# andfoy/py-distributed-dot-product

Hardware: AMD Instinct MI355X
Metric: ms/fwd+bwd DistributedDotProductAttn T=25000 d=768 h=8; scaling 1/2/4/8 GPU (lower is better)
Workload: dtype bf16; 1 GPU; model=DistributedDotProductAttn(d=768,h=8), global_batch=1, seq_len=25000, parallelism=sp1, impl=flash, mask=zeros, step=fwd+bwd+grad-allreduce+AdamW, launch=eager

## Files before the change

### csrc/bindings.cpp

```cpp
#include "bindings_common.h"

#include <algorithm>
#include <cmath>
#include <string>
#include <vector>

extern "C" const char xdot_build_id[];

using namespace xdot::bind;

namespace {

std::string build_id() { return std::string(xdot_build_id + 14); }

at::Tensor softmax_fwd(const at::Tensor& x, const c10::optional<at::Tensor>& mask, double scale,
                       int64_t mdiv, int64_t mmul, int64_t mmod) {
  Range rr_("xdot.softmax_fwd");
  TORCH_CHECK(x.is_cuda() && x.is_contiguous(), "xdot.softmax_fwd: x must be a contiguous GPU tensor");
  const int64_t T = x.size(-1);
  const int64_t rows = T == 0 ? 0 : x.numel() / T;
  auto y = at::empty_like(x);
  xdot::smx::Args a{};
  a.x = x.data_ptr(); a.out = y.data_ptr(); a.rows = rows; a.T = T; a.scale = (float)scale;
  a.mdiv = mdiv; a.mmul = mmul; a.mmod = mmod; a.mask = nullptr;
// ... 342 lines not shown
    hipKernelNodeAttrValue v{};
    v.priority = (int)prio;
    graph_ok(hipGraphKernelNodeSetAttribute(nd, hipKernelNodeAttributePriority, &v), "graph_set_kernel_priority");
    return;
  }
  TORCH_CHECK(false, "xdot.graph_set_kernel_priority: no kernel node ", index);
}

}

TORCH_LIBRARY(xdot, m) {
  m.def("gemm(Tensor A, Tensor B, Tensor(a!) C, int M, int N, int K, int nseg, int nb1, int nb2, "
        "int lda, int ldb, int ldc, int sA1, int sA2, int sB1, int sB2, int sC1, int sC2, "
        "int sAseg, int sBseg, bool a_mc, bool b_mc, float alpha, float beta=0.0, int path=0) -> ()");
  m.def("gemm_plan(int M, int N, int K, int nseg, int nb1, int nb2, int lda, int ldb, int ldc, int sA1, int sA2, "
        "int sB1, int sB2, int sC1, int sC2, int sAseg, int sBseg, bool a_mc, bool b_mc, float beta, ScalarType dt_in, "
        "ScalarType dt_out, bool a16, bool b16, bool c16, int path) -> int[]");
  m.def("softmax_fwd(Tensor x, Tensor? mask, float scale, int mdiv, int mmul, int mmod) -> Tensor");
  m.def("softmax_bwd(Tensor y, Tensor dy, float scale) -> Tensor");
  m.def("mask_pack(Tensor mask) -> (Tensor, Tensor, Tensor)");
  m.def("mask_gen(int B, int R, int T, bool causal, int window, int row_offset, Tensor? lengths, Tensor segs, Tensor? doc_starts=None, Tensor? row_runs=None) -> (Tensor, Tensor, Tensor)");
  m.def("flash_fwd(Tensor rows, Tensor kc, Tensor vc, Tensor? bits, Tensor? flags, int H, float scale, int nsplit=0, bool prescaled=False, int fp32_mode=0, Tensor(a!)? sbuf=None, int Hg=0) -> (Tensor, Tensor)");
  m.def("flash_bwd_cols(Tensor dout, Tensor rows, Tensor kc, Tensor vc, Tensor out, Tensor lse, Tensor? bits, "
        "Tensor? flags, int H, float scale, Tensor? delta=None, bool fp32_out=True, bool prescaled=False, "
        "Tensor? lse2=None, int fp32_mode=0, Tensor(a!)? sbuf=None, Tensor(b!)? dsbuf=None, int passes=3, "
        "Tensor(c!)? dkv_out=None, int Hg=0) -> (Tensor, Tensor)");
  m.def("flash_bwd_prep(Tensor dout, Tensor out, Tensor lse, int H) -> (Tensor, Tensor)");
  m.def("flash_bwd_delta(Tensor dout, Tensor out, int H) -> Tensor");
  m.def("sum_partials(Tensor part, ScalarType out_dtype) -> Tensor");
  m.def("flash_splits(int B, int R, int T, int H, bool rows_kernel) -> int");
  m.def("flash_fwd_plan(int B, int R, int T, int H, int D, ScalarType dtype, int fp32_mode, bool sbuf, int nsplit) -> int[]");
  m.def("flash_cols_plan(int B, int R, int T, int H, int D, ScalarType dtype, int fp32_mode, bool sbuf, bool dsbuf, "
        "int passes, bool prescaled, bool fp32_out, int Hg=0) -> int[]");
  m.def("flash_fwd_partial(Tensor rows, Tensor kc, Tensor vc, Tensor? bits, Tensor? flags, int H, float scale, "
        "Tensor(a!) opart, Tensor(b!) lpart, int sp0, int nsplit, bool prescaled=False, int fp32_mode=0, int Hg=0) -> ()");
  m.def("flash_fwd_combine(Tensor opart, Tensor lpart, int H, Tensor like) -> (Tensor, Tensor)");
  m.def("flash_bwd_rows_partial(Tensor dout, Tensor rows, Tensor kc, Tensor vc, Tensor lse, Tensor delta, Tensor? bits, "
        "Tensor? flags, int H, float scale, Tensor(a!) dpart, int sp0, int nsplit, bool prescaled=False, int fp32_mode=0, int Hg=0) -> ()");
  m.def("flash_bwd_rows_sum(Tensor dpart, int H, Tensor like) -> Tensor");
  m.def("flash_fwd_merge(Tensor(a!) opart, Tensor lpart, Tensor(b!) lrun, int H) -> ()");
  m.def("sum_partials_into(Tensor part, Tensor(a!) out) -> ()");
  m.def("cast_multi(Tensor[] src, Tensor(a!)[] dst) -> ()");
  m.def("adamw_step(Tensor(a!)[] params, Tensor[] grads, Tensor(b!)[] exp_avg, Tensor(c!)[] exp_avg_sq, float lr, "
        "float beta1, float beta2, float eps, float weight_decay, int step, Tensor[] step_ts, Tensor? lr_t, "
        "Tensor(d!)[] grad_out) -> ()");
  m.def("flash_bwd_rows(Tensor dout, Tensor rows, Tensor kc, Tensor vc, Tensor lse, Tensor delta, Tensor? bits, "
        "Tensor? flags, int H, float scale, int nsplit=0, bool prescaled=False, int fp32_mode=0, Tensor? sbuf=None, "
        "Tensor? dsbuf=None, int Hg=0) -> Tensor");
  m.def("flash_prescale(Tensor x, float scale) -> Tensor");
  m.def("rope_table(int R, int D, int offset, Tensor inv_freq) -> (Tensor, Tensor)");
  m.def("rope_apply(Tensor x, Tensor cos, Tensor sin, int H, bool inverse, float alpha, Tensor(a!) out) -> ()");
  m.def("headnorm_plan(int B, int R, int H, int D, ScalarType dtype) -> int[]");
  m.def("headnorm_fwd(Tensor x, Tensor weight, Tensor? cos, Tensor? sin, int H, float eps, float alpha, Tensor(a!) out, "
        "bool save) -> (Tensor, Tensor)");
  m.def("headnorm_bwd(Tensor g, Tensor x, Tensor rstd, Tensor weight, Tensor? cos, Tensor? sin, int H, float alpha, "
        "Tensor(a!) dx, bool need_dw) -> Tensor");
  m.def("sink_fold(Tensor(a!) out, Tensor(b!) lse, Tensor sinks, int H) -> ()");
  m.def("sink_grad(Tensor delta, Tensor lse, Tensor sinks) -> Tensor");
  m.def("gate_apply(Tensor o, Tensor g, int H, Tensor(a!) out, int mode=-1) -> ()");
  m.def("gate_backward(Tensor dy, Tensor o, Tensor g, int H, Tensor(a!) dout, int mode=-1) -> Tensor");
  m.def("mse_fwd(Tensor y, Tensor t) -> (Tensor, Tensor)");
  m.def("proj(Tensor x, Tensor w, Tensor? bias, bool nn, Tensor(a!)? out=None, int force=0, float alpha=1.0) -> Tensor");
  m.def("wgrad(Tensor dy, Tensor x, ScalarType out_dtype, int splits=0) -> Tensor");
  m.def("wgrad2(Tensor dy0, Tensor x0, Tensor dy1, Tensor x1, ScalarType out_dtype) -> Tensor[]");
  m.def("ipc_info() -> int[]");
  m.def("ipc_alloc(int nbytes, bool uncached) -> int");
// ... 43 lines not shown
```

### csrc/bindings_flash.cpp

```cpp
#include "bindings_common.h"
#include "flash_plan.h"

#include <vector>

namespace {

using namespace xdot::bind;
using namespace xdot::fa;
using OptT = c10::optional<at::Tensor>;

struct FlashGeom { int64_t B, R, C, T, D, ld, Cg, G; };

FlashGeom flash_check(const at::Tensor& rows, const at::Tensor& kc, const at::Tensor& vc, int64_t H, const OptT& bits,
                      const OptT& flags, bool colmajor = false, int64_t Hg = 0) {
  TORCH_CHECK(rows.is_cuda() && kc.is_cuda() && vc.is_cuda(), "xdot.flash: GPU tensors required");
  TORCH_CHECK(rows.is_contiguous(), "xdot.flash: rows must be contiguous");
  TORCH_CHECK(rows.scalar_type() == kc.scalar_type() && rows.scalar_type() == vc.scalar_type(), "xdot.flash: dtype mismatch");
  TORCH_CHECK(rows.scalar_type() == at::kBFloat16 || rows.scalar_type() == at::kHalf || rows.scalar_type() == at::kFloat,
              "xdot.flash: bf16/fp16/fp32 only");
  TORCH_CHECK(rows.dim() == 3 && kc.dim() == 3 && vc.sizes() == kc.sizes(), "xdot.flash: rows (B,R,C), cols (B,T,C)");
  FlashGeom g{rows.size(0), rows.size(1), rows.size(2), kc.size(1), 0, kc.stride(1), 0, 1};
  TORCH_CHECK(H > 0 && g.C % H == 0, "xdot.flash: C not divisible by heads");
  const int64_t hg = Hg > 0 ? Hg : H;
  TORCH_CHECK(hg <= H && H % hg == 0, "xdot.flash: the heads H = ", H, " must be a multiple of the gathered heads Hg = ", hg);
// ... 324 lines not shown
  Range rr_("xdot.flash_bwd_delta");
  return std::get<0>(bwd_prep(dout, out, nullptr, H, "flash_bwd_delta"));
}

std::tuple<at::Tensor, at::Tensor> flash_bwd_prep(const at::Tensor& dout, const at::Tensor& out, const at::Tensor& lse,
                                                  int64_t H) {
  Range rr_("xdot.flash_bwd_prep");
  return bwd_prep(dout, out, &lse, H, "flash_bwd_prep");
}

at::Tensor flash_bwd_rows(const at::Tensor& dout, const at::Tensor& rows, const at::Tensor& kc, const at::Tensor& vc,
                          const at::Tensor& lse, const at::Tensor& delta, const OptT& bits, const OptT& flags, int64_t H,
                          double scale, int64_t nsplit, bool prescaled, int64_t fp32_mode, const OptT& sbuf,
                          const OptT& dsbuf, int64_t Hg) {
  Range rr_("xdot.flash_bwd_rows");
  const FlashGeom g = flash_check(rows, kc, vc, H, bits, flags, false, Hg);
  float* sb = sbuf_ptr(sbuf, g, H, rows, fp32_mode, "xdot.flash_bwd_rows");
  float* dsb = sbuf_ptr(dsbuf, g, H, rows, fp32_mode, "xdot.flash_bwd_rows (dS buffer)");
  TORCH_CHECK(!dsb || sb || g.D <= 128, "xdot.flash_bwd_rows: a dS buffer without the score buffer needs D <= 128");
  check_bhr(delta, g.B, H, g.R, rows.device(), "xdot.flash_bwd_rows: delta");
  auto a = bwd_args(g, dout, rows, kc, vc, lse, bits, flags, H, scale, prescaled, fp32_mode);
  auto drows = at::empty_like(rows);
  const int ns = plan_rows(g, H, rows.scalar_type(), fp32_mode, sb || dsb, sb != nullptr, nsplit);
  at::Tensor dpart;
  if (ns > 1) dpart = at::empty({ns, g.B, g.R, g.C}, rows.options().dtype(at::kFloat));
  a.delta = delta.data_ptr<float>(); a.drows = drows.data_ptr();
  a.nsplit = ns; a.dpart = ns > 1 ? dpart.data_ptr<float>() : nullptr;
  a.sbuf = sb; a.dsbuf = dsb;
  c10::DeviceGuard guard(rows.device());
  launched(xdot_flash_bwd_rows_launch(&a, dt_code(rows.scalar_type()), (int)g.D, cur_stream(rows)), "flash_bwd_rows");
  return drows;
}

int64_t flash_splits(int64_t B, int64_t R, int64_t T, int64_t H, bool rows_kernel) {
  if (rows_kernel) return rows_split(B, R, T, H);
  return pick_split(((R + 127) / 128) * B * H, T, 512, 0);
}

void flash_fwd_partial(const at::Tensor& rows, const at::Tensor& kc, const at::Tensor& vc, const OptT& bits,
                       const OptT& flags, int64_t H, double scale, at::Tensor& opart, at::Tensor& lpart, int64_t sp0,
                       int64_t nsplit, bool prescaled, int64_t fp32_mode, int64_t Hg) {
  Range rr_("xdot.flash_fwd_partial");
  const FlashGeom g = flash_check(rows, kc, vc, H, bits, flags, false, Hg);
  TORCH_CHECK(sp0 >= 0 && nsplit >= 1, "xdot.flash_fwd_partial: slots");
  const int ns = pick_split(1, g.T, 1, nsplit);
  check_part(opart, sp0 + ns, g.B * g.R * g.C, "opart");
  check_part(lpart, sp0 + ns, g.B * H * g.R, "lpart");
  auto a = fwd_args(g, rows, kc, vc, bits, flags, H, scale, prescaled, fp32_mode);
  a.nsplit = ns; a.sp0 = (int)sp0; a.force_partial = 1;
  a.opart = opart.data_ptr<float>(); a.lpart = lpart.data_ptr<float>();
  c10::DeviceGuard guard(rows.device());
  launched(xdot_flash_fwd_launch(&a, dt_code(rows.scalar_type()), (int)g.D, cur_stream(rows)), "flash_fwd_partial");
}

void combine(xdot::fa::FwdArgs& a, const at::Tensor& opart, const at::Tensor& lpart, int64_t B, int64_t H, int64_t R,
             int64_t C, int dt, const char* op) {
  const int64_t S = opart.size(0);
  check_part(opart, S, B * R * C, "opart");
  check_part(lpart, S, B * H * R, "lpart");
  a.B = (int)B; a.H = (int)H; a.R = (int)R; a.nsplit = (int)S;
  a.opart = opart.data_ptr<float>(); a.lpart = lpart.data_ptr<float>();
  c10::DeviceGuard guard(opart.device());
  launched(xdot_flash_fwd_combine_launch(&a, dt, (int)(C / H), cur_stream(opart)), op);
}

std::tuple<at::Tensor, at::Tensor> flash_fwd_combine(const at::Tensor& opart, const at::Tensor& lpart, int64_t H,
// ... 29 lines not shown
  const FlashGeom g = flash_check(rows, kc, vc, H, bits, flags, false, Hg);
  check_bhr(delta, g.B, H, g.R, rows.device(), "xdot.flash_bwd_rows_partial: delta");
  TORCH_CHECK(sp0 >= 0 && nsplit >= 1, "xdot.flash_bwd_rows_partial: slots");
  const int ns = pick_split(1, g.T, 1, nsplit);
  check_part(dpart, sp0 + ns, g.B * g.R * g.C, "dpart");
  auto a = bwd_args(g, dout, rows, kc, vc, lse, bits, flags, H, scale, prescaled, fp32_mode);
  a.delta = delta.data_ptr<float>();
  a.nsplit = ns; a.sp0 = (int)sp0; a.force_partial = 1; a.dpart = dpart.data_ptr<float>();
  c10::DeviceGuard guard(rows.device());
  launched(xdot_flash_bwd_rows_launch(&a, dt_code(rows.scalar_type()), (int)g.D, cur_stream(rows)),
           "flash_bwd_rows_partial");
}

at::Tensor flash_bwd_rows_sum(const at::Tensor& dpart, int64_t H, const at::Tensor& like) {
  Range rr_("xdot.flash_bwd_rows_sum");
  const int64_t B = like.size(0), R = like.size(1), C = like.size(2), S = dpart.size(0);
  check_part(dpart, S, B * R * C, "dpart");
  auto out = at::empty_like(like);
  xdot::fa::BwdArgs a{};
  a.drows = out.data_ptr(); a.dpart = dpart.data_ptr<float>();
  a.B = (int)B; a.H = (int)H; a.R = (int)R; a.nsplit = (int)S;
  c10::DeviceGuard guard(like.device());
  launched(xdot_flash_bwd_rows_sum_launch(&a, dt_code(like.scalar_type()), (int)(C / H), cur_stream(like)),
           "flash_bwd_rows_sum");
  return out;
}

}

TORCH_LIBRARY_IMPL(xdot, CompositeExplicitAutograd, m) {
  m.impl("flash_splits", &flash_splits);
  m.impl("flash_fwd_plan", &flash_fwd_plan);
  m.impl("flash_cols_plan", &flash_cols_plan);
}

TORCH_LIBRARY_IMPL(xdot, CUDA, m) {
  m.impl("flash_fwd", &flash_fwd);
  m.impl("flash_bwd_cols", &flash_bwd_cols);
  m.impl("flash_bwd_rows", &flash_bwd_rows);
  m.impl("flash_bwd_delta", &flash_bwd_delta);
  m.impl("flash_bwd_prep", &flash_bwd_prep);
  m.impl("sum_partials", &sum_partials);
  m.impl("sum_partials_into", &sum_partials_into);
  m.impl("flash_prescale", &flash_prescale);
  m.impl("flash_fwd_partial", &flash_fwd_partial);
  m.impl("flash_fwd_combine", &flash_fwd_combine);
  m.impl("flash_fwd_merge", &flash_fwd_merge);
  m.impl("flash_bwd_rows_partial", &flash_bwd_rows_partial);
  m.impl("flash_bwd_rows_sum", &flash_bwd_rows_sum);
}
```

### csrc/flash_bwd.hip

```cpp
#include "flash_launch.h"

#include <algorithm>
#include <cstdlib>
#include <cstring>

#include <type_traits>

namespace xdot {
namespace fa {

template <int DT, int D>
__global__ __launch_bounds__(256) void flash_bwd_prep_kernel(BwdArgs a, const void* out_, float* delta) {
  using T16 = typename dt_traits<DT>::T;
  const int64_t idx = (int64_t)blockIdx.x * blockDim.x + threadIdx.x;
  const int64_t total = (int64_t)a.B * a.R * a.H;
  if (idx >= total) return;
  const int h = (int)(idx % a.H);
  const int64_t br = idx / a.H;
  const int row = (int)(br % a.R), b = (int)(br / a.R);
  const int64_t li = ((int64_t)b * a.H + h) * a.R + row;
  if (a.lse2) a.lse2[li] = a.lse[li] * LOG2E;
  if (!delta) return;
  const int64_t off = br * (a.H * D) + h * D;
  const T16* o = reinterpret_cast<const T16*>(out_) + off;
  const T16* d = reinterpret_cast<const T16*>(a.dout) + off;
  float acc = 0.f;
#pragma unroll
  for (int c = 0; c < D / 8; ++c) {
    union { u32x4 u; T16 e[8]; } x, y;
    x.u = *reinterpret_cast<const u32x4*>(o + 8 * c);
    y.u = *reinterpret_cast<const u32x4*>(d + 8 * c);
#pragma unroll
    for (int e = 0; e < 8; ++e) acc += (float)x.e[e] * (float)y.e[e];
  }
  delta[li] = acc;
// ... 537 lines not shown
template <int DT, int D>
static void launch_bwd_delta(const BwdArgs& a, const void* out, float* delta, hipStream_t st) {
  const int64_t n0 = (int64_t)a.B * a.R * a.H;
  if constexpr (D % 32 == 0 && D <= 128) {
    hipLaunchKernelGGL((flash_bwd_prep8_kernel<DT, D>), dim3((unsigned)((8 * n0 + 255) / 256)), dim3(256), 0, st, a, out,
                       delta);
    return;
  }
  hipLaunchKernelGGL((flash_bwd_prep_kernel<DT, D>), dim3((unsigned)((n0 + 255) / 256)), dim3(256), 0, st, a, out, delta);
}

template <int DT, int D>
static void launch_bwd_cols(const BwdArgs& a, hipStream_t st) {
  if (D <= 96 && a.prescaled && xdot_flash_bwd_cols2_launch(&a, DT, D, st) == 0) return;
  const int ncb = (a.T + 127) / 128;
  constexpr int LDS2 = 2 * ColsCfg<D, 2>::STAGE;
  if (a.G > 1) {
    const dim3 ggrid(ncb * a.B * (a.H / a.G));
    if (a.prescaled) hipLaunchKernelGGL((flash_bwd_cols_kernel<DT, D, 2, 2, true, true>), ggrid, dim3(256), LDS2, st, a);
    else hipLaunchKernelGGL((flash_bwd_cols_kernel<DT, D, 2, 2, false, true>), ggrid, dim3(256), LDS2, st, a);
    return;
  }
  const dim3 grid(ncb * a.B * a.H);
  if (a.prescaled) hipLaunchKernelGGL((flash_bwd_cols_kernel<DT, D, 2, 2, true>), grid, dim3(256), LDS2, st, a);
  else hipLaunchKernelGGL((flash_bwd_cols_kernel<DT, D, 2, 2>), grid, dim3(256), LDS2, st, a);
}

template <int DT, int D>
static void launch_rows_sum(const BwdArgs& a, hipStream_t st) {
  const int64_t n4 = (int64_t)a.B * a.R * a.H * D / 4;
  hipLaunchKernelGGL((flash_bwd_rows_sum<DT, D>), dim3((unsigned)((n4 + 255) / 256)), dim3(256), 0, st, a);
}

template <int DT, int D>
static void launch_bwd_rows(const BwdArgs& a, hipStream_t st) {
  const int nrb = (a.R + 127) / 128;
  constexpr int LDS = RowsCfg<D>::NBUF * RowsCfg<D>::STAGE;
  const dim3 grid(nrb * a.B * a.H * a.nsplit);
  if (a.prescaled) hipLaunchKernelGGL((flash_bwd_rows_kernel<DT, D, true>), grid, dim3(256), LDS, st, a);
  else hipLaunchKernelGGL((flash_bwd_rows_kernel<DT, D, false>), grid, dim3(256), LDS, st, a);
  if (a.nsplit > 1 && !a.force_partial) launch_rows_sum<DT, D>(a, st);
}

}
}

extern "C" int xdot_flash_bwd_delta_launch(const xdot::fa::BwdArgs* a, const void* out, float* delta, int dt, int D,
                                           hipStream_t st) {
  using namespace xdot;
  using namespace xdot::fa;
  if (a->R == 0 || a->B == 0 || a->H == 0) return 0;
  if (dt == DT_F32) return xdot_flash_bwd_prep_f32_launch(a, out, delta, D, st);
  return for_dtype16_any_head_dim(dt, D, -1, [&](auto t, auto d) {
    launch_bwd_delta<decltype(t)::value, decltype(d)::value>(*a, out, delta, st);
    return 0;
  });
}

extern "C" int xdot_flash_bwd_cols_launch(const xdot::fa::BwdArgs* a, int dt, int D, hipStream_t st) {
  using namespace xdot;
  using namespace xdot::fa;
  if (a->R == 0 || a->B == 0 || a->H == 0 || a->T == 0) return 0;
  if (D > 128) return xdot_flash_wide_cols_launch(a, dt, D, st);
  if (dt == DT_F32) return a->fp32_mode ? xdot_flash_bwd_cols_x3_launch(a, D, st) : xdot_flash_bwd_cols_f32_launch(a, D, st);
  return for_dtype16_head_dim(dt, D, -1, [&](auto t, auto d) {
    launch_bwd_cols<decltype(t)::value, decltype(d)::value>(*a, st);
    return 0;
  });
}

extern "C" int xdot_flash_cols_splits(const xdot::fa::BwdArgs* a, int dt, int D, int* sq, int* sv) {
  *sq = *sv = 1;
  if (a->R == 0 || a->B == 0 || a->H == 0 || a->T == 0) return 0;
  if (D > 128) {
    const int64_t W = (int64_t)((a->T + 127) / 128) * a->B * a->H, nrt = (a->R + 31) / 32;
// ... 33 lines not shown
  switch (dt) {
    case DT_F32: hipLaunchKernelGGL(fa::cols_sum_kernel<DT_F32>, grid, dim3(256), 0, st, part, out, S, rows, C, ldo); return 0;
    case DT_BF16: hipLaunchKernelGGL(fa::cols_sum_kernel<DT_BF16>, grid, dim3(256), 0, st, part, out, S, rows, C, ldo); return 0;
    case DT_F16: hipLaunchKernelGGL(fa::cols_sum_kernel<DT_F16>, grid, dim3(256), 0, st, part, out, S, rows, C, ldo); return 0;
    default: return -1;
  }
}

extern "C" int xdot_flash_bwd_rows_sum_launch(const xdot::fa::BwdArgs* a, int dt, int D, hipStream_t st) {
  using namespace xdot;
  using namespace xdot::fa;
  if (a->R == 0 || a->B == 0 || a->H == 0) return 0;
  if (dt == DT_F32) return xdot_flash_rows_sum_f32_launch(a, D, st);
  return for_dtype16_any_head_dim(dt, D, -1, [&](auto t, auto d) {
    launch_rows_sum<decltype(t)::value, decltype(d)::value>(*a, st);
    return 0;
  });
}

extern "C" int xdot_flash_bwd_rows_launch(const xdot::fa::BwdArgs* a, int dt, int D, hipStream_t st) {
  using namespace xdot;
  using namespace xdot::fa;
  if (a->R == 0 || a->B == 0 || a->H == 0 || a->T == 0) return 0;
  if (D > 128) {
    const int rc = xdot_flash_wide_rows_launch(a, dt, D, st);
    if (rc == 0 && a->nsplit > 1 && !a->force_partial) return xdot_flash_bwd_rows_sum_launch(a, dt, D, st);
    return rc;
  }
  if (dt == DT_F32) {
    const int rc = a->fp32_mode ? xdot_flash_bwd_rows_x3_launch(a, D, st) : xdot_flash_bwd_rows_f32_launch(a, D, st);
    if (rc == 0 && a->nsplit > 1 && !a->force_partial) return xdot_flash_rows_sum_f32_launch(a, D, st);
    return rc;
  }
  return for_dtype16_head_dim(dt, D, -1, [&](auto t, auto d) {
    launch_bwd_rows<decltype(t)::value, decltype(d)::value>(*a, st);
    return 0;
  });
}
```

### csrc/flash_launch.h

```cpp
#pragma once
#include "flash_common.h"

namespace xdot {
namespace fa {

template <auto Kernel, int LDS> int resident_wgs() {
  static const int v = [] {
    int n = 0;
    if (hipOccupancyMaxActiveBlocksPerMultiprocessor(&n, reinterpret_cast<const void*>(Kernel), 256, LDS) != hipSuccess || n < 1)
      n = 1;
    return n;
  }();
  return v;
}

template <class Args> struct Kern {
  void (*fn)(Args) = nullptr;
  int lds = 0;
  int (*occ)() = nullptr;
  explicit operator bool() const { return fn != nullptr; }
  void launch(dim3 grid, hipStream_t st, const Args& a) const {
    void* args[] = {const_cast<Args*>(&a)};
    (void)hipLaunchKernel(reinterpret_cast<const void*>(fn), grid, dim3(256), args, (size_t)lds, st);
  }
  int wgs_per_cu() const { return occ ? occ() : 0; }
  int slots() const { return wgs_per_cu() * xdot_num_cus(); }
};
template <class A> A kern_args(void (*)(A));
template <auto Kernel, int LDS> auto kern() {
  using K = Kern<decltype(kern_args(Kernel))>;
  if constexpr (LDS > 160 * 1024) return K{};
  else return K{Kernel, LDS, &resident_wgs<Kernel, LDS>};
}

template <class R, class F> R for_head_dim(int D, R none, F&& f) {
  switch (D) {
    case 32: return f(Ic<32>{});
    case 64: return f(Ic<64>{});
    case 96: return f(Ic<96>{});
    case 128: return f(Ic<128>{});
    default: return none;
  }
}
template <class R, class F> R for_wide_head_dim(int D, R none, F&& f) {
  switch (D) {
    case 160: return f(Ic<160>{});
    case 192: return f(Ic<192>{});
    case 256: return f(Ic<256>{});
    case 384: return f(Ic<384>{});
    default: return none;
  }
}
template <class R, class F> R for_dtype16_head_dim(int dt, int D, R none, F&& f) {
  switch (dt) {
    case DT_BF16: return for_head_dim(D, none, [&](auto d) -> R { return f(Ic<DT_BF16>{}, d); });
    case DT_F16: return for_head_dim(D, none, [&](auto d) -> R { return f(Ic<DT_F16>{}, d); });
    default: return none;
  }
}
template <class R, class F> R for_dtype16_any_head_dim(int dt, int D, R none, F&& f) {
  if (D <= 128) return for_dtype16_head_dim(dt, D, none, f);
  switch (dt) {
    case DT_BF16: return for_wide_head_dim(D, none, [&](auto d) -> R { return f(Ic<DT_BF16>{}, d); });
    case DT_F16: return for_wide_head_dim(D, none, [&](auto d) -> R { return f(Ic<DT_F16>{}, d); });
    default: return none;
// ... 36 lines not shown
```

### csrc/flash_plan.h

```cpp
#pragma once
#include <algorithm>
#include <cstdint>
#include <cstdlib>
#include <cstring>

namespace xdot {
namespace fa {

inline int env_int(const char* name, int lo, int hi = INT32_MAX) {
  const char* e = std::getenv(name);
  if (!e || !*e || !std::strcmp(e, "auto")) return -1;
  return std::max(lo, std::min(hi, std::atoi(e)));
}

inline bool f32_heavy() {
  const char* e = std::getenv("XDOT_F32_HEAVY");
  return !(e && e[0] == '0');
}

inline int pick_split(int64_t blocks, int64_t T, int64_t slots, int64_t req) {
  const int64_t nkt = (T + 63) / 64;
  if (req > 0) return (int)std::max<int64_t>(1, std::min<int64_t>(req, nkt));
  int best = 1;
  double best_cost = 1e300;
  for (int s = 1; s <= 8; ++s) {
    if (s > 1 && nkt / s < 8) break;
    const int64_t rounds = (blocks * s + slots - 1) / slots;
    const double cost = (double)rounds * ((double)nkt / s + 8.0);
    if (cost < best_cost * 0.985) { best_cost = cost; best = s; }
  }
  return best;
}

inline int rows_split(int64_t B, int64_t R, int64_t T, int64_t H) {
  const int64_t nkt = (T + 63) / 64, nrt = (R + 63) / 64;
  const int base = pick_split(((R + 127) / 128) * B * H, T, 512, 0);
  int64_t conc = (nkt * 36 + nrt * 48 - 1) / (nrt * 48);
  conc = std::min<int64_t>(8, std::max<int64_t>(1, std::min<int64_t>(conc, nkt / 8)));
  return std::max(base, (int)conc);
}

inline int pick_csplit(int64_t W, int nrt, int slots, int maxs, double per) {
  int best = 1;
  double bc = 1e300;
  for (int s = 1; s <= maxs && (s == 1 || nrt / s >= 16); ++s) {
    const double c = (double)((W * s + slots - 1) / slots) / s * (1.0 + per * (s - 1));
    if (c < bc * 0.98) {
      bc = c;
      best = s;
    }
  }
  return best;
}

inline int csplit_cols(int64_t W, int n, int slots) { return pick_csplit(W, n, slots, 4, 0.02); }
inline int csplit_f32_fwd(int64_t W, int n, int slots) { return pick_csplit(W, n, slots, 32, 0.001); }
inline int csplit_f32_rows(int64_t W, int n, int slots) { return pick_csplit(W, n, slots, 8, 0.004); }
inline int csplit_wide_rows(int64_t W, int n, int slots) { return pick_csplit(W, n, slots, 8, 0.01); }

inline bool head_heavy_plan(int64_t W, int64_t ntiles, int64_t S, int su, int* whole, int* rem, int* split) {
  if (W % 8 || S <= 0 || su <= 0) return false;
  const int64_t m = W / 8, full = m / S, r = m % S;
  if (r == 0 || full == 0) return false;
  const double cu = (double)((W * su + 8 * S - 1) / (8 * S)) * ((double)ntiles / su + 8.0);
  double best = 1e300;
  int bs = 0;
  for (int s = 1; s <= 16; ++s) {
    if (s > 1 && ntiles / s < 8) break;
    const double c = (double)full * ((double)ntiles + 8.0) + (double)((r * s + S - 1) / S) * ((double)ntiles / s + 8.0);
    if (c < best * 0.985) { best = c; bs = s; }
  }
  if (bs < 2 || best >= cu * 0.97) return false;
  *whole = (int)(full * S); *rem = (int)r; *split = bs;
  return true;
// ... 5 lines not shown
```

### csrc/kernels.h

```cpp
#pragma once
#include <hip/hip_runtime.h>
#include <stdint.h>

namespace xdot {

enum DType : int { DT_F32 = 0, DT_BF16 = 1, DT_F16 = 2 };

struct GemmArgs {
  const void* A;
  const void* B;
  void* C;
  int M, N, K;
  int nseg;
  int nb2;
  int tiles_m, tiles_n;
  int64_t lda, ldb, ldc;
  int64_t sA1, sA2, sB1, sB2, sC1, sC2;
  int64_t sAseg, sBseg;
  float alpha;
  float beta;
};

namespace smx {
struct Args {
// ... 187 lines not shown
}
}

extern "C" {
int xdot_gemm_launch(const xdot::GemmArgs* a, int batches, int dt_in, int dt_out, int a_mc,
                     int b_mc, int vec, hipStream_t st);
int xdot_gemm_f32_launch(const xdot::GemmArgs* a, int batches, int a_mc, int b_mc, int vec, hipStream_t st);
int xdot_gemm2_launch(const xdot::GemmArgs* a, int batches, int dt_in, int dt_out, int a_mc, int b_mc,
                      int splits, float* ws, hipStream_t st);
int xdot_gemm2_f32_launch(const xdot::GemmArgs* a, int batches, int a_mc, int b_mc, int splits, float* ws,
                          hipStream_t st);
int xdot_num_cus();
int xdot_gemm_reduce_launch(const xdot::GemmArgs* a, const float* ws, int splits, int batches, int dt_out,
                            hipStream_t st);
int xdot_gemm3_launch(const xdot::GemmArgs* a, int batches, int dt_in, int dt_out, int a_mc, int b_mc,
                      int splits, float* ws, hipStream_t st);
int xdot_gemm_proj_launch(const xdot::ProjArgs* a, int dt, int nn, int force, hipStream_t st);
int xdot_gemm_wgrad_launch(int np, const void* const* A, const void* const* B, float* const* part, const int* M,
                           const int* N, const int* K, const int* S, const int64_t* lda, const int64_t* ldb, int dt,
                           hipStream_t st);
int xdot_split3_launch(const float* src, void* dst, int64_t s1, int64_t s2, int64_t sseg, int64_t ld,
                       int nb1, int nb2, int nseg, int R, int C, int lo_mask, hipStream_t st);
int xdot_softmax_fwd_launch(const xdot::smx::Args* a, int dt, int vec, hipStream_t st);
int xdot_softmax_bwd_launch(const xdot::smx::Args* a, int dt, int vec, hipStream_t st);
int xdot_mask_pack_launch(const uint8_t* mask, uint64_t* bits, uint64_t* bt, uint8_t* flags, int B, int R, int T,
                          hipStream_t st);
int xdot_mask_gen_launch(uint64_t* bits, uint64_t* bt, uint8_t* flags, const int* lengths, const int* segs, int nseg,
                         int causal, int64_t window, int64_t row_off, int B, int R, int T, const int* starts, int nstarts,
                         int64_t starts_stride, const int* rows, int nrows, hipStream_t st);
int xdot_flash_fwd_launch(const xdot::fa::FwdArgs* a, int dt, int D, hipStream_t st);
int xdot_flash_bwd_delta_launch(const xdot::fa::BwdArgs* a, const void* out, float* delta, int dt, int D, hipStream_t st);
int xdot_flash_bwd_cols_launch(const xdot::fa::BwdArgs* a, int dt, int D, hipStream_t st);
int xdot_flash_bwd_rows_launch(const xdot::fa::BwdArgs* a, int dt, int D, hipStream_t st);
int xdot_flash_bwd_cols2_launch(const xdot::fa::BwdArgs* a, int dt, int D, hipStream_t st);
int xdot_sum_partials_launch(const float* part, void* out, int S, int64_t n, int dto, hipStream_t st);
int xdot_sum_partials2_launch(const float* pa, void* oa, int Sa, int64_t na, const float* pb, void* ob, int Sb,
                              int64_t nb, int dto, hipStream_t st);
int xdot_prescale_rows_launch(const void* x, void* out, int64_t n, float scale, int dt, hipStream_t st);
int xdot_rope_table_launch(float* cos, float* sin, const double* inv_freq, int R, int half, int64_t offset,
                           hipStream_t st);
int xdot_rope_apply_launch(const xdot::RopeArgs* a, int dt, int mode, hipStream_t st);
int xdot_headnorm_plan(int B, int R, int H, int D, int esize, xdot::HeadNormPlan* p);
int xdot_headnorm_fwd_launch(const xdot::HeadNormArgs* a, int dt, int vec, hipStream_t st);
int xdot_headnorm_bwd_launch(const xdot::HeadNormArgs* a, int dt, int vec, hipStream_t st);
int xdot_headnorm_dw_launch(const float* part, void* dw, int nparts, int D, int dto, hipStream_t st);
int xdot_sink_fold_launch(const xdot::SinkArgs* a, int dt, hipStream_t st);
int xdot_sink_grad_parts(int B, int R);
int xdot_sink_grad_launch(const xdot::SinkGradArgs* a, hipStream_t st);
int xdot_gate_apply_launch(const xdot::GateArgs* a, int dt, int vec, hipStream_t st);
int xdot_gate_backward_launch(const xdot::GateArgs* a, int dt, int vec, hipStream_t st);
int xdot_flash_fwd_rows_per_wg();
int xdot_adamw_launch(const xdot::AdamArgs* a, int dt, hipStream_t st);
int xdot_flash_f32_fwd_occ(int D, bool sbuf);
int xdot_cast_multi_launch(const xdot::CastArgs* a, hipStream_t st);
int xdot_mse_fwd_launch(const void* y, const void* t, void* dy, float* part, int nparts, void* loss, int64_t n, int dt,
                        hipStream_t st);
int xdot_flash_fwd_combine_launch(const xdot::fa::FwdArgs* a, int dt, int D, hipStream_t st);
int xdot_flash_bwd_rows_sum_launch(const xdot::fa::BwdArgs* a, int dt, int D, hipStream_t st);
int xdot_flash_fwd_f32_launch(const xdot::fa::FwdArgs* a, int D, hipStream_t st);
int xdot_flash_combine_f32_launch(const xdot::fa::FwdArgs* a, int D, hipStream_t st);
int xdot_flash_bwd_prep_f32_launch(const xdot::fa::BwdArgs* a, const void* out, float* delta, int D, hipStream_t st);
int xdot_flash_bwd_rows_f32_launch(const xdot::fa::BwdArgs* a, int D, hipStream_t st);
int xdot_flash_bwd_cols_f32_launch(const xdot::fa::BwdArgs* a, int D, hipStream_t st);
int xdot_flash_cols_splits(const xdot::fa::BwdArgs* a, int dt, int D, int* sq, int* sv);
int xdot_flash_cols_splits_f32(const xdot::fa::BwdArgs* a, int D, int* sq, int* sv);
int xdot_flash_cols_splits_x3(const xdot::fa::BwdArgs* a, int D, int* sq, int* sv);
// ... 30 lines not shown
```

Measured before the change: 7.815 ms.

## Add 16x16x32 MFMA variant of flash backward rows kernel for large grids

Adds a new dQ (rows) backward attention kernel built on 16x16x32 bf16/fp16 MFMA instructions, with its own LDS fragment addressing, transposed LDS reads and interleaved exp/pack scheduling. It is only available for head dims 64 and 96. It is picked automatically when the row-block grid has at least 512 workgroups, and can be forced either way with an environment variable. The aim is better MFMA utilisation and softmax/matmul overlap in the rows pass. In exchange it adds a second kernel path with separate masking and lane-mapping logic, a plan-query binding and a launch counter.

Result: no change. 7.833 ms (+0.2%).

```diff
diff --git a/csrc/bindings.cpp b/csrc/bindings.cpp
--- a/csrc/bindings.cpp
+++ b/csrc/bindings.cpp
@@ -398,6 +398,9 @@
   m.def("flash_fwd_plan(int B, int R, int T, int H, int D, ScalarType dtype, int fp32_mode, bool sbuf, int nsplit) -> int[]");
   m.def("flash_cols_plan(int B, int R, int T, int H, int D, ScalarType dtype, int fp32_mode, bool sbuf, bool dsbuf, "
         "int passes, bool prescaled, bool fp32_out, int Hg=0) -> int[]");
+  m.def("flash_rows_plan(int B, int R, int T, int H, int D, ScalarType dtype, int fp32_mode, bool sbuf, bool dsbuf, "
+        "int nsplit, bool prescaled) -> int[]");
+  m.def("flash_rows16_launches() -> int");
   m.def("flash_fwd_partial(Tensor rows, Tensor kc, Tensor vc, Tensor? bits, Tensor? flags, int H, float scale, "
         "Tensor(a!) opart, Tensor(b!) lpart, int sp0, int nsplit, bool prescaled=False, int fp32_mode=0, int Hg=0) -> ()");
   m.def("flash_fwd_combine(Tensor opart, Tensor lpart, int H, Tensor like) -> (Tensor, Tensor)");
diff --git a/csrc/bindings_flash.cpp b/csrc/bindings_flash.cpp
--- a/csrc/bindings_flash.cpp
+++ b/csrc/bindings_flash.cpp
@@ -380,6 +380,15 @@
   return drows;
 }
 
+std::vector<int64_t> flash_rows_plan(int64_t B, int64_t R, int64_t T, int64_t H, int64_t D, at::ScalarType dtype,
+                                     int64_t fp32_mode, bool sbuf, bool dsbuf, int64_t nsplit, bool prescaled) {
+  const int ns = plan_rows(query_geom(B, R, T, H, D), H, dtype, fp32_mode, sbuf || dsbuf, sbuf, nsplit);
+  const int mfma = dtype == at::kFloat ? 0 : xdot_flash_rows_mfma(dt_code(dtype), (int)D, prescaled, B, R, H);
+  return {ns, mfma};
+}
+
+int64_t flash_rows16_launches() { return xdot_flash_rows16_launches(); }
+
 int64_t flash_splits(int64_t B, int64_t R, int64_t T, int64_t H, bool rows_kernel) {
   if (rows_kernel) return rows_split(B, R, T, H);
   return pick_split(((R + 127) / 128) * B * H, T, 512, 0);
@@ -475,6 +484,8 @@
   m.impl("flash_splits", &flash_splits);
   m.impl("flash_fwd_plan", &flash_fwd_plan);
   m.impl("flash_cols_plan", &flash_cols_plan);
+  m.impl("flash_rows_plan", &flash_rows_plan);
+  m.impl("flash_rows16_launches", &flash_rows16_launches);
 }
 
 TORCH_LIBRARY_IMPL(xdot, CUDA, m) {
diff --git a/csrc/flash_bwd.hip b/csrc/flash_bwd.hip
--- a/csrc/flash_bwd.hip
+++ b/csrc/flash_bwd.hip
@@ -1,6 +1,7 @@
 #include "flash_launch.h"
 
 #include <algorithm>
+#include <atomic>
 #include <cstdlib>
 #include <cstring>
 
@@ -604,15 +605,15 @@
   hipLaunchKernelGGL((flash_bwd_rows_sum<DT, D>), dim3((unsigned)((n4 + 255) / 256)), dim3(256), 0, st, a);
 }
 
-template <int DT, int D>
-static void launch_bwd_rows(const BwdArgs& a, hipStream_t st) {
-  const int nrb = (a.R + 127) / 128;
-  constexpr int LDS = RowsCfg<D>::NBUF * RowsCfg<D>::STAGE;
-  const dim3 grid(nrb * a.B * a.H * a.nsplit);
-  if (a.prescaled) hipLaunchKernelGGL((flash_bwd_rows_kernel<DT, D, true>), grid, dim3(256), LDS, st, a);
-  else hipLaunchKernelGGL((flash_bwd_rows_kernel<DT, D, false>), grid, dim3(256), LDS, st, a);
-  if (a.nsplit > 1 && !a.force_partial) launch_rows_sum<DT, D>(a, st);
-}
+Kern<BwdArgs> rows32_kern(int dt, int D, bool prescaled) {
+  return for_dtype16_head_dim(dt, D, Kern<BwdArgs>{}, [&](auto t, auto d) {
+    constexpr int DT = decltype(t)::value, DV = decltype(d)::value;
+    constexpr int LDS = RowsCfg<DV>::NBUF * RowsCfg<DV>::STAGE;
+    return prescaled ? kern<flash_bwd_rows_kernel<DT, DV, true>, LDS>() : kern<flash_bwd_rows_kernel<DT, DV, false>, LDS>();
+  });
+}
+
+static std::atomic<int64_t> rows16_launches{0};
 
 }
 }
@@ -712,8 +713,18 @@
     if (rc == 0 && a->nsplit > 1 && !a->force_partial) return xdot_flash_rows_sum_f32_launch(a, D, st);
     return rc;
   }
-  return for_dtype16_head_dim(dt, D, -1, [&](auto t, auto d) {
-    launch_bwd_rows<decltype(t)::value, decltype(d)::value>(*a, st);
-    return 0;
-  });
-}
+  int mfma = 32;
+  const auto k = rows_kern(dt, D, a->prescaled != 0, rows_mfma(a->B, a->R, a->H), &mfma);
+  if (!k) return -1;
+  k.launch(dim3((unsigned)(((a->R + 127) / 128) * a->B * a->H * a->nsplit)), st, *a);
+  if (mfma == 16) rows16_launches.fetch_add(1, std::memory_order_relaxed);
+  if (a->nsplit > 1 && !a->force_partial) return xdot_flash_bwd_rows_sum_launch(a, dt, D, st);
+  return 0;
+}
+
+extern "C" int xdot_flash_rows_mfma(int dt, int D, int prescaled, int64_t B, int64_t R, int64_t H) {
+  int mfma = 0;
+  if (D > 128 || !xdot::fa::rows_kern(dt, D, prescaled != 0, xdot::fa::rows_mfma(B, R, H), &mfma)) return 0;
+  return mfma;
+}
+extern "C" int64_t xdot_flash_rows16_launches() { return xdot::fa::rows16_launches.load(std::memory_order_relaxed); }
diff --git a/csrc/flash_launch.h b/csrc/flash_launch.h
--- a/csrc/flash_launch.h
+++ b/csrc/flash_launch.h
@@ -31,6 +31,14 @@
   using K = Kern<decltype(kern_args(Kernel))>;
   if constexpr (LDS > 160 * 1024) return K{};
   else return K{Kernel, LDS, &resident_wgs<Kernel, LDS>};
+}
+
+Kern<BwdArgs> rows32_kern(int dt, int D, bool prescaled);
+Kern<BwdArgs> rows16_kern(int dt, int D, bool prescaled);
+inline Kern<BwdArgs> rows_kern(int dt, int D, bool prescaled, int want, int* mfma = nullptr) {
+  Kern<BwdArgs> k = want == 16 ? rows16_kern(dt, D, prescaled) : Kern<BwdArgs>{};
+  if (mfma) *mfma = k ? 16 : 32;
+  return k ? k : rows32_kern(dt, D, prescaled);
 }
 
 template <class R, class F> R for_head_dim(int D, R none, F&& f) {
diff --git a/csrc/flash_plan.h b/csrc/flash_plan.h
--- a/csrc/flash_plan.h
+++ b/csrc/flash_plan.h
@@ -40,6 +40,12 @@
   return std::max(base, (int)conc);
 }
 
+inline int rows_mfma(int64_t B, int64_t R, int64_t H) {
+  const int e = env_int("XDOT_ROWS_MFMA", 16, 32);
+  if (e >= 0) return e == 16 ? 16 : 32;
+  return ((R + 127) / 128) * B * H >= 512 ? 16 : 32;
+}
+
 inline int pick_csplit(int64_t W, int nrt, int slots, int maxs, double per) {
   int best = 1;
   double bc = 1e300;
diff --git a/csrc/flash_rows16.hip b/csrc/flash_rows16.hip
--- /dev/null
+++ b/csrc/flash_rows16.hip
@@ -0,0 +1,322 @@
+#include "flash_launch.h"
+
+namespace xdot {
+namespace fa {
+
+template <int DT> struct mfma16;
+template <> struct mfma16<DT_BF16> {
+  static __device__ __forceinline__ f32x4 run(u32x4 a, u32x4 b, f32x4 c) {
+    return __builtin_amdgcn_mfma_f32_16x16x32_bf16(__builtin_bit_cast(bf16x8, a), __builtin_bit_cast(bf16x8, b), c, 0, 0, 0);
+  }
+};
+template <> struct mfma16<DT_F16> {
+  static __device__ __forceinline__ f32x4 run(u32x4 a, u32x4 b, f32x4 c) {
+    return __builtin_amdgcn_mfma_f32_16x16x32_f16(__builtin_bit_cast(f16x8, a), __builtin_bit_cast(f16x8, b), c, 0, 0, 0);
+  }
+};
+
+__device__ __forceinline__ int kchunk(int g) { return (4 - g) & 3; }
+
+struct Lanes16 {
+  int rb;
+  int tb0, tb1;
+};
+template <int D>
+__device__ __forceinline__ Lanes16 make_lanes16(int lane) {
+  constexpr int ROW = Img<D>::ROW;
+  Lanes16 L;
+  const int g = lane >> 4, i = lane & 15, q = i >> 2, p = i & 3;
+  L.rb = i * ROW + ((kchunk(g) ^ q) << 4);
+  L.tb0 = (4 * g + q) * ROW + (((p >> 1) ^ g) << 4) + 8 * (p & 1);
+  L.tb1 = (4 * g + q) * ROW + (((2 + (p >> 1)) ^ g) << 4) + 8 * (p & 1);
+  return L;
+}
+template <int D>
+__device__ __forceinline__ u32x4 row_frag16(const char* img, int r0, int ks, const Lanes16& L) {
+  return *reinterpret_cast<const u32x4*>(img + L.rb + r0 * Img<D>::ROW + ks * 64);
+}
+template <int D>
+__device__ __forceinline__ u32x4 tr_frag16(const char* img, int k0, int m, const Lanes16& L) {
+  constexpr int ROW = Img<D>::ROW;
+  typedef const __attribute__((address_space(3))) char lds_char;
+  lds_char* base = (lds_char*)img + ((m & 1) ? L.tb1 : L.tb0);
+  s16x4 lo = __builtin_amdgcn_ds_read_tr16_b64_v4i16((lds_s16x4*)(base + (k0 * ROW + (m >> 1) * 64)));
+  s16x4 hi = __builtin_amdgcn_ds_read_tr16_b64_v4i16((lds_s16x4*)(base + ((k0 + 16) * ROW + (m >> 1) * 64)));
+  union { struct { s16x4 a, b; } s; u32x4 u; } c;
+  c.s.a = lo;
+  c.s.b = hi;
+  return c.u;
+}
+
+__device__ __forceinline__ uint64_t tile_bits16(uint64_t w, int valid, int g) {
+  if (valid < 64) w |= ~0ull << valid;
+  return w >> (4 * g);
+}
+template <int B0>
+__device__ __forceinline__ void sel_bits4(f32x4& d, uint32_t w, uint32_t ybits) {
+  d[0] = sel_bit<B0 + 0>(w, d[0], ybits);
+  d[1] = sel_bit<B0 + 1>(w, d[1], ybits);
+  d[2] = sel_bit<B0 + 2>(w, d[2], ybits);
+  d[3] = sel_bit<B0 + 3>(w, d[3], ybits);
+}
+
+struct Sub16 { f32x4 t[2][2]; };
+
+template <int DT, int D, bool PS = false>
+__global__ __launch_bounds__(256, 2) void flash_bwd_rows16_kernel(BwdArgs a) {
+  using T16 = typename dt_traits<DT>::T;
+  using CF = RowsCfg<D>;
+  constexpr int IMG = CF::IMG, NG = CF::NG, PF = CF::PF, NBUF = CF::NBUF;
+  constexpr int KS = D / 32, MB = D / 16;
+
+  const int tid = threadIdx.x, lane = tid & 63, g4 = lane >> 4, i16 = lane & 15;
+  const int wave = __builtin_amdgcn_readfirstlane(tid >> 6);
+  const Lanes16 L = make_lanes16<D>(lane);
+  const int nrb = (a.R + 127) / 128;
+  const int lin = xcd_remap(blockIdx.x, gridDim.x);
+  const int rb = lin % nrb, bhs = lin / nrb;
+  const int bh = bhs % (a.B * a.H), sp = bhs / (a.B * a.H);
+  const int b = bh / a.H, h = bh % a.H;
+  const int C = a.H * D;
+  const int NKT = (a.T + 63) / 64;
+  const int kt_beg = (int)((int64_t)sp * NKT / a.nsplit), kt_end = (int)((int64_t)(sp + 1) * NKT / a.nsplit);
+  const int r0 = rb * 128 + wave * 32;
+  const int row[2] = {r0 + i16, r0 + 16 + i16};
+  const bool row_ok[2] = {row[0] < a.R, row[1] < a.R};
+
+  u32x4 kf[2][KS], df[2][KS];
+  float lse2[2], dlt[2];
+#pragma unroll
+  for (int nb = 0; nb < 2; ++nb) {
+    const int64_t off = ((int64_t)b * a.R + row[nb]) * C + h * D + 8 * kchunk(g4);
+    const T16* pk = reinterpret_cast<const T16*>(a.rows) + off;
+    const T16* pd = reinterpret_cast<const T16*>(a.dout) + off;
+#pragma unroll
+    for (int s = 0; s < KS; ++s) {
+      kf[nb][s] = row_ok[nb] ? *reinterpret_cast<const u32x4*>(pk + 32 * s) : u32x4{0, 0, 0, 0};
+      df[nb][s] = row_ok[nb] ? *reinterpret_cast<const u32x4*>(pd + 32 * s) : u32x4{0, 0, 0, 0};
+    }
+    const int64_t lrow = ((int64_t)b * a.H + h) * a.R + (row_ok[nb] ? row[nb] : 0);
+    lse2[nb] = row_ok[nb] ? a.lse[lrow] * LOG2E : 0.f;
+    dlt[nb] = row_ok[nb] ? a.delta[lrow] : 0.f;
+  }
+#pragma unroll
+  for (int nb = 0; nb < 2; ++nb) {
+#pragma unroll
+    for (int s = 0; s < KS; ++s) asm volatile("" : "+v"(kf[nb][s]), "+v"(df[nb][s]));
+    asm volatile("" : "+v"(lse2[nb]), "+v"(dlt[nb]));
+  }
+  const float c2 = a.scale * LOG2E;
+  f32x4 dseed[2], sseed[2];
+#pragma unroll
+  for (int nb = 0; nb < 2; ++nb) {
+#pragma unroll
+    for (int s = 0; s < KS; ++s) df[nb][s] ^= u32x4{0x80008000u, 0x80008000u, 0x80008000u, 0x80008000u};
+    const float sv = PS ? -lse2[nb] : 0.f;
+    dseed[nb] = f32x4{dlt[nb], dlt[nb], dlt[nb], dlt[nb]};
+    sseed[nb] = f32x4{sv, sv, sv, sv};
+  }
+
+  const int ldb = a.ldkv * 2;
+  ImgDma<D> dma;
+  dma.init(wave, lane, ldb);
+  const int hg = a.G > 1 ? (h * a.gmul) >> 20 : h;
+  const char* kcb = reinterpret_cast<const char*>(reinterpret_cast<const T16*>(a.kc) + hg * D + (int64_t)b * a.T * a.ldkv);
+  const char* vcb = reinterpret_cast<const char*>(reinterpret_cast<const T16*>(a.vc) + hg * D + (int64_t)b * a.T * a.ldkv);
+  const uint64_t* mwg = a.mbits ? a.mbits + (int64_t)b * NKT * a.R + rb * 128 : nullptr;
+  const uint32_t moff = (uint32_t)(min((wave & 1) * 64 + lane, a.R - 1 - rb * 128) * 8 + (wave >> 1) * 4);
+  const int NKT4 = (NKT + 3) & ~3;
+  const int NRB32 = (a.R + 31) / 32;
+  const uint8_t* fwg = a.mflags ? a.mflags + ((int64_t)b * NRB32 + rb * 4) * NKT4 : nullptr;
+  const int fn = min(4, NRB32 - rb * 4);
+  auto issue = [&](int kt) {
+    char* st = smem + ((kt - kt_beg) % NBUF) * CF::STAGE;
+    const int64_t t0 = (int64_t)kt * 64;
+    const int rmax = a.T - 1 - (int)t0;
+    dma.issue(kcb + t0 * ldb, ldb, rmax, st, wave);
+    dma.issue(vcb + t0 * ldb, ldb, rmax, st + IMG, wave);
+    if (mwg) {
+      glds4(mwg + (int64_t)kt * a.R, moff, st + CF::OFF_W + (wave >> 1) * 512 + (wave & 1) * 256);
+      glds_flags(fwg, NKT4, fn, kt >> 2, st + CF::OFF_F);
+    } else {
+      glds4(kcb, (uint32_t)lane * 4, st + CF::OFF_X);
+      glds4(kcb, (uint32_t)lane * 4, st + CF::OFF_X);
+    }
+  };
+
+  f32x4 dk[MB][2];
+#pragma unroll
+  for (int m = 0; m < MB; ++m)
+#pragma unroll
+    for (int nb = 0; nb < 2; ++nb) dk[m][nb] = f32x4{0.f, 0.f, 0.f, 0.f};
+
+  auto seeds = [&](bool masked, uint64_t w0, uint64_t w1, int tt) {
+    Sub16 sd;
+#pragma unroll
+    for (int nb = 0; nb < 2; ++nb) {
+      sd.t[0][nb] = sseed[nb];
+      sd.t[1][nb] = sseed[nb];
+      if (masked) {
+        const uint32_t w = (uint32_t)((nb ? w1 : w0) >> (32 * tt));
+        sel_bits4<0>(sd.t[0][nb], w, NINF_BITS);
+        sel_bits4<16>(sd.t[1][nb], w, NINF_BITS);
+      }
+    }
+    return sd;
+  };
+  auto pipe_body = [&](const char* qs, const char* vs, bool masked, uint64_t w0, uint64_t w1) __attribute__((always_inline)) {
+    constexpr int NA = 8 * KS, NP = NA / 2;
+    constexpr int GK = 3 * MB;
+    auto elem = [&](Sub16& sc, const Sub16& dc, u32x4 (&pk)[2], int e) {
+      const int nb = e >> 3, mbl = (e >> 2) & 1, r = e & 3;
+      const float x = PS ? sc.t[mbl][nb][r] : __builtin_fmaf(sc.t[mbl][nb][r], c2, -lse2[nb]);
+      float y = fast_exp2(x) * dc.t[mbl][nb][r];
+      asm volatile("" : "+v"(y));
+      sc.t[mbl][nb][r] = y;
+      if (e & 1) {
+        uint32_t w = pack2<DT>(sc.t[mbl][nb][r - 1], y);
+        asm volatile("" : "+v"(w));
+        pk[nb][(e & 7) >> 1] = w;
+      }
+    };
+    auto opnd = [&](int tt, int p) {
+      return row_frag16<D>((p & 1) ? vs : qs, tt * 32 + 16 * ((p >> 1) & 1), p >> 2, L);
+    };
+    auto chain = [&](Sub16& s, Sub16& d, const Sub16& sd, const u32x4& o, int i) {
+      const int nb = i & 1, p = i >> 1, ks = p >> 2, mbl = (p >> 1) & 1;
+      if (p & 1) d.t[mbl][nb] = mfma16<DT>::run(o, df[nb][ks], ks == 0 ? dseed[nb] : d.t[mbl][nb]);
+      else s.t[mbl][nb] = mfma16<DT>::run(o, kf[nb][ks], ks == 0 ? sd.t[mbl][nb] : s.t[mbl][nb]);
+    };
+    Sub16 s0, d0, s1, d1;
+    u32x4 p0[2], p1[2];
+    const Sub16 sd0 = seeds(masked, w0, w1, 0);
+    const Sub16 sd1 = seeds(masked, w0, w1, 1);
+    {
+      u32x4 ow[NP];
+      ow[0] = opnd(0, 0);
+      ow[1] = opnd(0, 1);
+      __builtin_amdgcn_iglp_opt(1);
+#pragma unroll
+      for (int p = 0; p < NP; ++p) {
+        if (p + 2 < NP) ow[p + 2] = opnd(0, p + 2);
+        chain(s0, d0, sd0, ow[p], 2 * p);
+        chain(s0, d0, sd0, ow[p], 2 * p + 1);
+      }
+    }
+    u32x4 tq[MB];
+    {
+      u32x4 o0 = opnd(1, 0), o1 = opnd(1, 1);
+#pragma unroll
+      for (int p = 0; p < NP; ++p) {
+        u32x4 o2 = o1;
+        if (p + 2 < NP) o2 = opnd(1, p + 2);
+        if (p == NP - 1) tq[0] = tr_frag16<D>(qs, 0, 0, L);
+#pragma unroll
+        for (int i = 2 * p; i < 2 * p + 2; ++i) {
+          chain(s1, d1, sd1, o0, i);
+#pragma unroll
+          for (int e = (i * 16 + NA - 1) / NA; e < ((i + 1) * 16 + NA - 1) / NA; ++e) elem(s0, d0, p0, e);
+          __builtin_amdgcn_sched_barrier(0);
+        }
+        o0 = o1;
+        o1 = o2;
+      }
+    }
+    {
+      u32x4 tk[MB];
+#pragma unroll
+      for (int j = 0; j < GK; ++j) {
+        if (j < 2 * MB) {
+          const int m = j >> 1, nb = j & 1;
+          if (!nb) {
+            if (m + 1 < MB) tq[m + 1] = tr_frag16<D>(qs, 0, m + 1, L);
+            else tk[0] = tr_frag16<D>(qs, 32, 0, L);
+          }
+          dk[m][nb] = mfma16<DT>::run(tq[m], p0[nb], dk[m][nb]);
+        } else {
+          const int m = j - 2 * MB;
+          if (m + 1 < MB) tk[m + 1] = tr_frag16<D>(qs, 32, m + 1, L);
+          dk[m][0] = mfma16<DT>::run(tk[m], p1[0], dk[m][0]);
+        }
+#pragma unroll
+        for (int e = (j * 16 + GK - 1) / GK; e < ((j + 1) * 16 + GK - 1) / GK; ++e) elem(s1, d1, p1, e);
+        __builtin_amdgcn_sched_barrier(0);
+      }
+#pragma unroll
+      for (int m = 0; m < MB; ++m) dk[m][1] = mfma16<DT>::run(tk[m], p1[1], dk[m][1]);
+    }
+  };
+
+  auto tile = [&](auto bufc, int kt) {
+    constexpr int BUF = decltype(bufc)::value;
+    if (kt + PF < kt_end) issue(kt + PF);
+    const char* qs = smem + BUF * CF::STAGE;
+    const char* vs = qs + IMG;
+    const int flag = r0 >= a.R ? 1 : (fwg ? staged_flag(qs + CF::OFF_F, wave, kt & 3) : 0);
+    const bool tail = (kt + 1) * 64 > a.T;
+    if (flag != 1) {
+      if (flag == 2 || tail) {
+        const int valid = a.T - kt * 64;
+        const uint64_t w0 = tile_bits16(flag == 2 ? staged_word(qs + CF::OFF_W, wave * 32 + i16) : 0ull, valid, g4);
+        const uint64_t w1 = tile_bits16(flag == 2 ? staged_word(qs + CF::OFF_W, wave * 32 + 16 + i16) : 0ull, valid, g4);
+        pipe_body(qs, vs, true, w0, w1);
+      } else {
+        pipe_body(qs, vs, false, 0ull, 0ull);
+      }
+    }
+    if (kt + PF < kt_end) wait_vm<NG * (PF - 1)>();
+    else wait_vm<0>();
+    raw_barrier();
+  };
+
+#pragma unroll
+  for (int t = 0; t < PF; ++t)
+    if (kt_beg + t < kt_end) issue(kt_beg + t);
+  if (PF > 1 && kt_beg + 1 < kt_end) wait_vm<NG * (PF - 1)>();
+  else wait_vm<0>();
+  raw_barrier();
+  for (int kt = kt_beg; kt < kt_end; kt += NBUF) {
+    tile(std::integral_constant<int, 0>{}, kt);
+    if (kt + 1 < kt_end) tile(std::integral_constant<int, 1>{}, kt + 1);
+    if constexpr (NBUF > 2) {
+      if (kt + 2 < kt_end) tile(std::integral_constant<int, 2>{}, kt + 2);
+    }
+  }
+  const float nscale = -a.scale;
+  const bool partial = a.nsplit > 1 || a.force_partial;
+#pragma unroll
+  for (int nb = 0; nb < 2; ++nb) {
+    if (!row_ok[nb]) continue;
+    if (partial) {
+      float* op = a.dpart + (((int64_t)(a.sp0 + sp) * a.B + b) * a.R + row[nb]) * C + h * D + 4 * g4;
+#pragma unroll
+      for (int m = 0; m < MB; ++m) *reinterpret_cast<f32x4*>(op + 16 * m) = dk[m][nb] * nscale;
+    } else {
+      T16* op = reinterpret_cast<T16*>(a.drows) + ((int64_t)b * a.R + row[nb]) * C + h * D + 4 * g4;
+#pragma unroll
+      for (int m = 0; m < MB; ++m) {
+        u32x2 wv;
+        wv[0] = pack2<DT>(dk[m][nb][0] * nscale, dk[m][nb][1] * nscale);
+        wv[1] = pack2<DT>(dk[m][nb][2] * nscale, dk[m][nb][3] * nscale);
+        *reinterpret_cast<u32x2*>(op + 16 * m) = wv;
+      }
+    }
+  }
+}
+
+Kern<BwdArgs> rows16_kern(int dt, int D, bool prescaled) {
+  const auto pick = [&](auto t, auto d) -> Kern<BwdArgs> {
+    constexpr int DT = decltype(t)::value, DV = decltype(d)::value;
+    constexpr int LDS = RowsCfg<DV>::NBUF * RowsCfg<DV>::STAGE;
+    return prescaled ? kern<flash_bwd_rows16_kernel<DT, DV, true>, LDS>() : kern<flash_bwd_rows16_kernel<DT, DV, false>, LDS>();
+  };
+  if (D != 64 && D != 96) return {};
+  switch (dt) {
+    case DT_BF16: return D == 64 ? pick(Ic<DT_BF16>{}, Ic<64>{}) : pick(Ic<DT_BF16>{}, Ic<96>{});
+    case DT_F16: return D == 64 ? pick(Ic<DT_F16>{}, Ic<64>{}) : pick(Ic<DT_F16>{}, Ic<96>{});
+    default: return {};
+  }
+}
+
+}
+}
diff --git a/csrc/kernels.h b/csrc/kernels.h
--- a/csrc/kernels.h
+++ b/csrc/kernels.h
@@ -243,6 +243,8 @@
 int xdot_flash_bwd_delta_launch(const xdot::fa::BwdArgs* a, const void* out, float* delta, int dt, int D, hipStream_t st);
 int xdot_flash_bwd_cols_launch(const xdot::fa::BwdArgs* a, int dt, int D, hipStream_t st);
 int xdot_flash_bwd_rows_launch(const xdot::fa::BwdArgs* a, int dt, int D, hipStream_t st);
+int xdot_flash_rows_mfma(int dt, int D, int prescaled, int64_t B, int64_t R, int64_t H);
+int64_t xdot_flash_rows16_launches();
 int xdot_flash_bwd_cols2_launch(const xdot::fa::BwdArgs* a, int dt, int D, hipStream_t st);
 int xdot_sum_partials_launch(const float* part, void* out, int S, int64_t n, int dto, hipStream_t st);
 int xdot_sum_partials2_launch(const float* pa, void* oa, int Sa, int64_t na, const float* pb, void* ob, int Sb,
```
